# OPPOMKLab/u-LLaVA

Hardware: AMD Instinct MI355X
Metric: images/sec/GPU (ViT-L-336 + LLaMA-7B + SAM RES forward) at 1/2/4/8 MI355X (higher is better)
Workload: dtype bf16; 1 GPU; C4: ViT-L/14-336 + LLaMA-7B instruct forward, 336x336 image + 64-token prompt (S=643), batch 32/GPU; per_gpu_batch=32, global_batch=32, seq_len=643, image=336, parallelism=dp1, weights=random-init N(0,0.02), ViT-L/14 + LLaMA-7B (V=32011) shapes

## Files before the change

### u-llava_amd/csrc/gemm.hip

```cpp
#include "ull_common.h"
#include <stdlib.h>
#include <type_traits>

namespace {

constexpr int BM = 128, BN = 128, BK = 64;
constexpr int TILE_BYTES = BM * BK * 2;
constexpr int BUF_BYTES = 2 * TILE_BYTES;
constexpr int GEMM_LDS = 2 * BUF_BYTES;
constexpr int GROUP_M = 8;

constexpr int EPI_BIAS = 1, EPI_ACT_SHIFT = 1, EPI_ACT_MASK = 3 << 1;
constexpr int EPI_RESID = 8, EPI_SWIGLU = 16, EPI_OUT_F32 = 32;
constexpr int EPI_W_TILED = 64, EPI_X_TILED = 128;
constexpr int EPI_BIAS_ROUNDED = 256;
constexpr int ULL_W4_FORCE_STAGED = 512;

struct GemmArgs {
    const elem_t* X; const elem_t* W; void* C;
    const elem_t* bias; const elem_t* R;
    long ldx, ldw, ldc, ldr;
    int M, N, K, flags;
    int nbm, nbn;
    int t_full, sk;
// ... 733 lines not shown
    __builtin_amdgcn_s_barrier();
    staged_epilogue<SWIGLU, 4>(p, acc, smem + wave * (64 * 144), lane, m0 + wm * 64, n0 + wn * 64);
}
#endif


struct PatchArgs {
    const elem_t* img; const elem_t* zeros; const elem_t* img_end;
    int C, H, W, ps, gw, gh;
    int nseg;
    int xcd_raster;
};

template <int DUMMY>
__global__ __launch_bounds__(256, 2) void patchify_gemm_kernel(GemmArgs p, PatchArgs q) {
    extern __shared__ __attribute__((aligned(16))) char smem[];
    const int tid = threadIdx.x;
    const int lane = tid & 63;
    const int wave = __builtin_amdgcn_readfirstlane(tid >> 6);
    const int wn = wave & 1, wm = wave >> 1;
    const int nwg = p.nbm * p.nbn;
    int bid = blockIdx.x;
    {
        const int qq = nwg >> 3, r = nwg & 7, xcd = bid & 7, k = bid >> 3;
        bid = (xcd < r ? xcd * (qq + 1) : r * (qq + 1) + (xcd - r) * qq) + k;
    }
    const int per_group = GROUP_M * p.nbn;
    const int gid = bid / per_group;
    const int first_m = gid * GROUP_M;
    const int gsz = min(p.nbm - first_m, GROUP_M);
    const int bm = first_m + (bid % per_group) % gsz;
    const int bn = (bid % per_group) / gsz;
    const int m0 = bm * BM, n0 = bn * BN;

    const int srow = lane >> 3;
    const int schunk = (lane & 7) ^ srow;
    const int seg = schunk >> 1, half = schunk & 1;
    const elem_t* xbase[4];
    const elem_t* wsrc[4];
#pragma unroll
    for (int i = 0; i < 4; ++i) {
        const int r = (wave * 4 + i) * 8 + srow;
        const int m = min(m0 + r, p.M - 1);
        const int px = m % q.gw, py = (m / q.gw) % q.gh, b = m / (q.gw * q.gh);
        xbase[i] = q.img + (((long)b * q.C * q.H + (long)py * q.ps) * q.W + px * q.ps) + half * 8;
        wsrc[i] = p.W + (long)min(n0 + r, p.N - 1) * p.ldw + schunk * 8;
    }
    const int stage_off = wave * 4 * 8 * (BK * 2);
    const uint32_t lds_base = __builtin_amdgcn_readfirstlane((uint32_t)(uintptr_t)(__attribute__((address_space(3))) char*)smem);
    auto stage = [&](int buf, int kt) {
        const uint32_t bx = lds_base + buf * BUF_BYTES + stage_off;
        const uint32_t bw = bx + TILE_BYTES;
        const int idx = kt * 4 + seg;
        const int c = idx / q.ps, ky = idx - c * q.ps;
        const long xoff = ((long)c * q.H + ky) * q.W;
        const bool real = idx < q.nseg;
        const long ko = (long)kt * BK;
#pragma unroll
        for (int i = 0; i < 4; ++i) {
            const elem_t* sp = real ? xbase[i] + xoff : q.zeros;
            if (real && sp + 8 > q.img_end) {
                const uint32_t* s32 = (const uint32_t*)sp;
                const uint4 v = make_uint4(s32[0], s32[1], s32[2], 0u);
                *(uint4*)(smem + buf * BUF_BYTES + stage_off + i * 1024 + lane * 16) = v;
                asm volatile("s_waitcnt lgkmcnt(0)" ::: "memory");
            } else {
                glds16(sp, bx + i * 1024);
            }
            glds16(wsrc[i] + ko, bw + i * 1024);
        }
    };

    const int frow = lane & 15, fgrp = lane >> 4;
    int swz[2];
    swz[0] = ((0 + fgrp) ^ (lane & 7)) << 4;
    swz[1] = ((4 + fgrp) ^ (lane & 7)) << 4;
    const int xrow_off = (wm * 64 + frow) * (BK * 2);
    const int wrow_off = TILE_BYTES + (wn * 64 + frow) * (BK * 2);

    f32x4_t acc[4][4];
#pragma unroll
    for (int i = 0; i < 4; ++i)
#pragma unroll
        for (int j = 0; j < 4; ++j) acc[i][j] = f32x4_t{0.f, 0.f, 0.f, 0.f};

    const int nk = p.K / BK;
    stage(0, 0);
    for (int kt = 0; kt < nk; ++kt) {
        const int cur = kt & 1;
        asm volatile("s_waitcnt vmcnt(0)" ::: "memory");
        __builtin_amdgcn_s_barrier();
        if (kt + 1 < nk) stage(cur ^ 1, kt + 1);
        const char* base = smem + cur * BUF_BYTES;
#pragma unroll
        for (int kk = 0; kk < 2; ++kk) {
            uint4 wf[4], xf[4];
#pragma unroll
            for (int i = 0; i < 4; ++i) wf[i] = *(const uint4*)(base + wrow_off + i * 16 * (BK * 2) + swz[kk]);
#pragma unroll
            for (int j = 0; j < 4; ++j) xf[j] = *(const uint4*)(base + xrow_off + j * 16 * (BK * 2) + swz[kk]);
#pragma unroll
            for (int i = 0; i < 4; ++i)
#pragma unroll
                for (int j = 0; j < 4; ++j) acc[i][j] = mfma16(wf[i], xf[j], acc[i][j]);
        }
    }
    __builtin_amdgcn_s_barrier();
    staged_epilogue<false, 4>(p, acc, smem + wave * (64 * 144), lane, m0 + wm * 64, n0 + wn * 64);
}

#define ULL_STAMP(slot) ((void)0)

namespace big {

constexpr int BM = 256, BN = 256, BK = 64;
constexpr int OP_BYTES = BM * BK * 2;
constexpr int SLOT_BYTES = 2 * OP_BYTES;
constexpr int LDS_BYTES = 8 * 128 * (64 * 2 + 16);
constexpr int LDS_BYTES_W4 = LDS_BYTES + 16 * 1024;

struct Frags { uint4 w[4]; uint4 x[8]; };

template <bool SWIGLU, bool ROPE = false>
__global__ __launch_bounds__(512) void gemm256_kernel(GemmArgs p) {
    extern __shared__ __attribute__((aligned(16))) char smem[];
    const int tid = threadIdx.x, lane = tid & 63;
    const int wave = __builtin_amdgcn_readfirstlane(tid >> 6);
    const int wn = wave & 3, wm = wave >> 2;
    int bid = blockIdx.x;
    int slice = 0;
    const bool split = bid >= p.t_full;
    if (!split) {
        const int nwg = p.t_full;
        const int q = nwg >> 3, r = nwg & 7, xcd = bid & 7, k = bid >> 3;
        bid = (xcd < r ? xcd * (q + 1) : r * (q + 1) + (xcd - r) * q) + k;
    } else {
        const int r = bid - p.t_full;
        bid = p.t_full + r / p.sk;
        slice = r % p.sk;
    }
    const int per_group = p.group_m * p.nbn;
    const int gid = bid / per_group;
    const int first_m = gid * p.group_m;
    const int gsz = min(p.nbm - first_m, p.group_m);
    const int bm = first_m + (bid % per_group) % gsz;
    const int bn = (bid % per_group) / gsz;
    const int m0 = bm * BM, n0 = bn * BN;
    const int nk_total = p.K / BK;
    const bool w_tiled = p.flags & EPI_W_TILED, x_tiled = p.flags & EPI_X_TILED;

    const int srow = lane >> 3;
    const int schunk = (lane & 7) ^ srow;
    const elem_t* xsrc[4];
    const elem_t* wsrc[4];
#pragma unroll
    for (int i = 0; i < 4; ++i) {
        const int r = (wave * 4 + i) * 8 + srow;
        xsrc[i] = x_tiled ? p.X + (((long)bm * nk_total) * BM + r) * BK + schunk * 8
                          : p.X + (long)min(m0 + r, p.M - 1) * p.ldx + schunk * 8;
        wsrc[i] = w_tiled ? p.W + (((long)bn * nk_total) * BN + r) * BK + schunk * 8
                          : p.W + (long)min(n0 + r, p.N - 1) * p.ldw + schunk * 8;
    }
    const long xstep = x_tiled ? BM * BK : BK, wstep = w_tiled ? BN * BK : BK;
    const uint32_t lds_base = __builtin_amdgcn_readfirstlane((uint32_t)(uintptr_t)(__attribute__((address_space(3))) char*)smem);
    const uint32_t piece_off = wave * 4 * 1024;
    auto stage = [&](int kt) {
        const uint32_t bx = lds_base + (kt & 1) * SLOT_BYTES + piece_off;
        const long kox = (long)kt * xstep, kow = (long)kt * wstep;
#pragma unroll
        for (int i = 0; i < 4; ++i) {
            glds16(xsrc[i] + kox, bx + i * 1024);
            glds16(wsrc[i] + kow, bx + OP_BYTES + i * 1024);
        }
    };

    const int fr = lane & 15, fg = lane >> 4;
    int swz[2];
    swz[0] = ((0 + fg) ^ (lane & 7)) << 4;
    swz[1] = ((4 + fg) ^ (lane & 7)) << 4;
    const int xoff = (wm * 128 + fr) * (BK * 2);
    const int woff = OP_BYTES + (wn * 64 + fr) * (BK * 2);
    auto read_frags = [&](int kt, int kk, Frags& f) {
        const char* base = smem + (kt & 1) * SLOT_BYTES + swz[kk];
#pragma unroll
        for (int i = 0; i < 4; ++i) f.w[i] = *(const uint4*)(base + woff + i * 16 * (BK * 2));
#pragma unroll
        for (int j = 0; j < 8; ++j) f.x[j] = *(const uint4*)(base + xoff + j * 16 * (BK * 2));
    };

    f32x4_t acc[4][8];
#pragma unroll
    for (int i = 0; i < 4; ++i)
#pragma unroll
        for (int j = 0; j < 8; ++j) acc[i][j] = f32x4_t{0.f, 0.f, 0.f, 0.f};
    int nk = p.K / BK;
    if (split) {
        const int kt0 = (int)((long)nk * slice / p.sk), kt1 = (int)((long)nk * (slice + 1) / p.sk);
#pragma unroll
        for (int i = 0; i < 4; ++i) { xsrc[i] += (long)kt0 * xstep; wsrc[i] += (long)kt0 * wstep; }
        nk = kt1 - kt0;
    }
constexpr int ULL_W8_BAR_A = 14;
constexpr int ULL_W8_DMA_STRIDE = 6;
constexpr int ULL_W8_BAR_B = 40;
constexpr int ULL_W8_FA_STRIDE = 2;
    constexpr int W8_BAR_A = ULL_W8_BAR_A, W8_DMA_STRIDE = ULL_W8_DMA_STRIDE, W8_BAR_B = ULL_W8_BAR_B, W8_FA_STRIDE = ULL_W8_FA_STRIDE;
    constexpr int W8_ISSUED = (W8_BAR_B - W8_BAR_A + W8_DMA_STRIDE - 1) / W8_DMA_STRIDE;
    constexpr int W8_INFLIGHT = W8_ISSUED > 8 ? 8 : W8_ISSUED;
    static_assert(W8_BAR_A >= 12 && W8_BAR_B >= W8_BAR_A && W8_BAR_A + 7 * W8_DMA_STRIDE < 64 && W8_BAR_B + 11 * W8_FA_STRIDE < 64, "schedule");
    constexpr int USE_ORDER[12] = {0, 4, 1, 2, 3, 5, 6, 7, 8, 9, 10, 11};
    auto read1 = [&](int kt, int kk, Frags& f, int r) {
        const char* base = smem + (kt & 1) * SLOT_BYTES + swz[kk];
        if (r < 4) f.w[r] = *(const uint4*)(base + woff + r * 16 * (BK * 2));
        else f.x[r - 4] = *(const uint4*)(base + xoff + (r - 4) * 16 * (BK * 2));
    };
    auto mma1 = [&](const Frags& f, int s) {
        const int j = s >> 2, i = s & 3;
        acc[i][j] = mfma16(f.w[i], f.x[j], acc[i][j]);
    };
    stage(0);
    stage(1);
    asm volatile("s_waitcnt vmcnt(8)" ::: "memory");
    __builtin_amdgcn_s_barrier();
    Frags fa, fb;
    read_frags(0, 0, fa);
    const uint32_t dump = lds_base + LDS_BYTES;
#pragma clang loop unroll(disable)
    for (int kt = 0; kt < nk; ++kt) {
        const bool with_dma = kt + 2 < nk;
        const int ktd = with_dma ? kt + 2 : nk - 1;
        const long kox = (long)ktd * xstep, kow = (long)ktd * wstep;
        const uint32_t bx = with_dma ? lds_base + (kt & 1) * SLOT_BYTES + piece_off : dump;
        const uint32_t bw = with_dma ? bx + OP_BYTES : dump + 4096;
#pragma clang loop unroll(full)
        for (int s = 0; s < 64; ++s) {
            if (s == W8_BAR_A) {
                asm volatile("s_waitcnt lgkmcnt(0)" ::: "memory");
                __builtin_amdgcn_s_barrier();
            }
            if (s == W8_BAR_B) {
                asm volatile("s_waitcnt vmcnt(%0)" :: "n"(W8_INFLIGHT) : "memory");
                __builtin_amdgcn_s_barrier();
            }
            if (s < 12) read1(kt, 1, fb, s);
            if (s >= W8_BAR_B && (s - W8_BAR_B) % W8_FA_STRIDE == 0 && (s - W8_BAR_B) / W8_FA_STRIDE < 12)
                read1(kt + 1, 0, fa, USE_ORDER[(s - W8_BAR_B) / W8_FA_STRIDE]);
            if (s >= W8_BAR_A && (s - W8_BAR_A) % W8_DMA_STRIDE == 0 && (s - W8_BAR_A) / W8_DMA_STRIDE < 8) {
                const int pc = (s - W8_BAR_A) / W8_DMA_STRIDE;
                if (pc < 4) glds16(xsrc[pc] + kox, bx + pc * 1024);
                else glds16(wsrc[pc - 4] + kow, bw + (pc - 4) * 1024);
            }
            mma1(s < 32 ? fa : fb, s & 31);
            __builtin_amdgcn_sched_barrier(0);
        }
    }

    if (split) {
        float* slab = p.ws + ((long)(bid - p.t_full) * p.sk + slice) * (BM * BN);
#pragma clang loop unroll(full)
        for (int j = 0; j < 8; ++j)
#pragma clang loop unroll(full)
            for (int i = 0; i < 4; ++i)
                *(f32x4_t*)(slab + (wm * 128 + j * 16 + fr) * BN + wn * 64 + i * 16 + fg * 4) = acc[i][j];
        return;
    }
    __builtin_amdgcn_s_barrier();
    staged_epilogue<SWIGLU, 8, ROPE>(p, acc, smem + wave * (128 * 144), lane, m0 + wm * 128, n0 + wn * 64, smem + (wave ^ 1) * (128 * 144));
}


struct Frags4 { uint4 w[8]; uint4 x[8]; };

#ifdef ULL_ELEM_F16
#define ULL_MFMA16_ASM "v_mfma_f32_16x16x32_f16"
#else
#define ULL_MFMA16_ASM "v_mfma_f32_16x16x32_bf16"
#endif
typedef uint32_t u32x4_t __attribute__((ext_vector_type(4)));
ULL_DEV void mfma16_inplace(f32x4_t& c, const uint4& a, const uint4& b) {
    const u32x4_t av = {a.x, a.y, a.z, a.w}, bv = {b.x, b.y, b.z, b.w};
    asm volatile(ULL_MFMA16_ASM " %0, %1, %2, %0" : "+a"(c) : "v"(av), "v"(bv));
}


template <bool SWIGLU> ULL_DEV int w4_row_swizzle(int row) {
    return SWIGLU ? (((row >> 1) & 1) | (((row >> 3) & 1) << 1) | (((row >> 5) & 1) << 2)) : (((row >> 1) & 1) | (((row >> 3) & 3) << 1));
}
template <bool SWIGLU> ULL_DEV constexpr int w4_frag_row(int c) {
    return SWIGLU ? 64 * (c >> 2) + 16 * (c & 1) + 4 * ((c >> 1) & 1) : 32 * (c >> 1) + 4 * (c & 1);
}
template <bool SWIGLU> ULL_DEV int w4_lane_row(int fr) {
    return SWIGLU ? 32 * (fr >> 3) + 8 * ((fr >> 2) & 1) + (fr & 3) : 8 * (fr >> 2) + (fr & 3);
}
template <bool SWIGLU> ULL_DEV int w4_acc_row(int h, int i, int fg) {
    return SWIGLU ? h * 64 + 32 * (fg >> 1) + 16 * (i & 1) + 8 * (fg & 1) + 4 * (i >> 1) : h * 64 + 32 * (i >> 1) + 8 * fg + 4 * (i & 1);
}

ULL_DEV f32x4_t w4_acc_to_vgpr(const f32x4_t& a) {
    f32x4_t t = a;
    asm volatile("" : "+v"(t));
    return t;
}

template <bool SWIGLU, bool ROPE, int NH = 2, int RPF = 8>
ULL_DEV void w4_direct_epilogue(const GemmArgs& p, f32x4_t (&acc)[NH][4][8], int lane, int mrow0, int nw0) {
    static_assert(NH == 2 || (!SWIGLU && !ROPE), "SwiGLU and RoPE pair columns across the two halves");
    const int fr = lane & 15, fg = lane >> 4;
    if constexpr (SWIGLU) {
        const int n_out = p.N / 2, nb = nw0 / 2 + 8 * fg;
        elem_t* cb = (elem_t*)p.C + nb;
#pragma clang loop unroll(full)
        for (int j = 0; j < 8; ++j) {
            const int m = mrow0 + j * 16 + fr;
#pragma clang loop unroll(full)
            for (int h = 0; h < 2; ++h) {
                float v[8];
#pragma clang loop unroll(full)
                for (int pp = 0; pp < 2; ++pp) {
                    const f32x4_t ag = w4_acc_to_vgpr(acc[h][2 * pp][j]), au = w4_acc_to_vgpr(acc[h][2 * pp + 1][j]);
#pragma unroll
                    for (int r = 0; r < 4; ++r) {
                        const float g = rnd(ag[r]);
                        const float u = rnd(au[r]);
                        v[4 * pp + r] = rnd(act_silu(g)) * u;
                    }
                }
                if (m < p.M && nb + h * 32 + 8 <= n_out) *(uint4*)(cb + (long)m * p.ldc + h * 32) = pack8(v);
            }
            __builtin_amdgcn_sched_barrier(0);
        }
    } else {
        const int flags = p.flags;
        const bool has_bias = flags & EPI_BIAS, has_res = flags & EPI_RESID;
        const bool rope_on = ROPE && nw0 < p.rope_cols;
        const int nb = nw0 + 8 * fg;
        uint4 bvp[NH][2];
#pragma unroll
        for (int h = 0; h < NH; ++h)
#pragma unroll
            for (int pp = 0; pp < 2; ++pp) {
                const int n = nb + h * 64 + pp * 32;
                bvp[h][pp] = (has_bias && n + 8 <= p.N) ? *(const uint4*)(p.bias + n) : uint4{0, 0, 0, 0};
            }
        elem_t* cb = (elem_t*)p.C + nb;
        const elem_t* rb = p.R + nb;
        auto body = [&](auto with_bias, auto with_res, auto act_kind) {
            constexpr bool WB = decltype(with_bias)::value, WR = decltype(with_res)::value;
            constexpr int ACT = decltype(act_kind)::value;
            constexpr int NB_ = ROPE ? 2 : RPF;
            uint4 rv[NB_][NH][2], tc[NB_][2], ts[NB_][2];
            auto fetch = [&](int j, int buf) {
                const long mc = min(mrow0 + j * 16 + fr, p.M - 1);
                if constexpr (WR) {
#pragma unroll
                    for (int h = 0; h < NH; ++h)
#pragma unroll
                        for (int pp = 0; pp < 2; ++pp) rv[buf][h][pp] = *(const uint4*)(rb + mc * p.ldr + h * 64 + pp * 32);
                }
                if constexpr (ROPE) {
                    if (rope_on) {
#pragma unroll
                        for (int pp = 0; pp < 2; ++pp) {
                            tc[buf][pp] = *(const uint4*)(p.rope_cos + mc * 64 + pp * 32 + 8 * fg);
                            ts[buf][pp] = *(const uint4*)(p.rope_sin + mc * 64 + pp * 32 + 8 * fg);
                        }
                    }
                }
            };
            if constexpr (ROPE || NB_ < 8) fetch(0, 0);
            else if constexpr (WR) {
#pragma clang loop unroll(full)
                for (int j = 0; j < 8; ++j) fetch(j, j);
                __builtin_amdgcn_sched_barrier(0);
            }
#pragma clang loop unroll(full)
            for (int j = 0; j < 8; ++j) {
                const int m = mrow0 + j * 16 + fr;
                if constexpr (ROPE || NB_ < 8) { if (j + 1 < 8) fetch(j + 1, (j + 1) % NB_); }
                uint4 o[NH][2];
#pragma unroll
                for (int h = 0; h < NH; ++h)
#pragma unroll
                    for (int pp = 0; pp < 2; ++pp) {
                        float v[8], bv[8];
                        if constexpr (WB) unpack8(bvp[h][pp], bv);
                        const f32x4_t a0 = w4_acc_to_vgpr(acc[h][2 * pp][j]), a1 = w4_acc_to_vgpr(acc[h][2 * pp + 1][j]);
#pragma unroll
                        for (int e = 0; e < 8; ++e) {
                            const float a = e < 4 ? a0[e & 3] : a1[e & 3];
                            v[e] = WB ? a + bv[e] : a;
                        }
                        o[h][pp] = pack8(v);
                        if constexpr (ACT != 0) {
                            float a[8];
                            unpack8(o[h][pp], a);
                            if constexpr (ACT == 2) {
#pragma unroll
                                for (int e = 0; e < 8; e += 2) {
                                    const f32x2_t r = act_gelu_erf2(f32x2_t{a[e], a[e + 1]});
                                    a[e] = r.x; a[e + 1] = r.y;
                                }
                            } else {
#pragma unroll
                                for (int e = 0; e < 8; ++e) a[e] = ACT == 1 ? act_quick_gelu_e(a[e]) : fmaxf(a[e], 0.f);
                            }
                            o[h][pp] = pack8(a);
                        }
                    }
                if constexpr (ROPE) {
                    if (rope_on) {
#pragma unroll
                        for (int pp = 0; pp < 2; ++pp) {
                            float x0[8], x1[8], cs[8], sn[8];
                            unpack8(o[0][pp], x0); unpack8(o[1][pp], x1);
                            unpack8(tc[j % NB_][pp], cs); unpack8(ts[j % NB_][pp], sn);
                            float y0[8], y1[8];
#pragma unroll
                            for (int e = 0; e < 8; ++e) {
                                y0[e] = rnd(x0[e] * cs[e]) + rnd(-x1[e] * sn[e]);
                                y1[e] = rnd(x1[e] * cs[e]) + rnd(x0[e] * sn[e]);
                            }
                            o[0][pp] = pack8(y0); o[1][pp] = pack8(y1);
                        }
                    }
                }
#pragma unroll
                for (int h = 0; h < NH; ++h)
#pragma unroll
                    for (int pp = 0; pp < 2; ++pp) {
                        if constexpr (WR) {
                            float a[8], b[8];
                            unpack8(o[h][pp], a); unpack8(rv[j % NB_][h][pp], b);
#pragma unroll
                            for (int e = 0; e < 8; ++e) a[e] = rnd(b[e] + a[e]);
                            o[h][pp] = pack8(a);
                        }
                        if (m < p.M && nb + h * 64 + pp * 32 + 8 <= p.N) *(uint4*)(cb + (long)m * p.ldc + h * 64 + pp * 32) = o[h][pp];
                    }
                __builtin_amdgcn_sched_barrier(0);
            }
        };
        using I0 = std::integral_constant<int, 0>;
        const int act = (flags & EPI_ACT_MASK) >> EPI_ACT_SHIFT;
        if constexpr (!ROPE) {
            if (act) {
                if (act == 1) { if (has_bias) body(std::true_type{}, std::false_type{}, std::integral_constant<int, 1>{}); else body(std::false_type{}, std::false_type{}, std::integral_constant<int, 1>{}); }
                else if (act == 2) { if (has_bias) body(std::true_type{}, std::false_type{}, std::integral_constant<int, 2>{}); else body(std::false_type{}, std::false_type{}, std::integral_constant<int, 2>{}); }
                else { if (has_bias) body(std::true_type{}, std::false_type{}, std::integral_constant<int, 3>{}); else body(std::false_type{}, std::false_type{}, std::integral_constant<int, 3>{}); }
                return;
            }
        }
        if (has_bias) { if (has_res) body(std::true_type{}, std::true_type{}, I0{}); else body(std::true_type{}, std::false_type{}, I0{}); }
        else { if (has_res) body(std::false_type{}, std::true_type{}, I0{}); else body(std::false_type{}, std::false_type{}, I0{}); }
    }
}

template <bool SWIGLU, bool ROPE = false>
__global__ __launch_bounds__(256) void gemm256w4_kernel(GemmArgs p) {
    extern __shared__ __attribute__((aligned(16))) char smem[];
    ULL_STAMP(0); ULL_STAMP(7);
    const int tid = threadIdx.x, lane = tid & 63;
    const int wave = __builtin_amdgcn_readfirstlane(tid >> 6);
    const int wn = wave & 1, wm = wave >> 1;
    int bid = blockIdx.x;
    int slice = 0;
    const bool split = bid >= p.t_full;
    if (!split) {
        const int nwg = p.t_full;
        const int q = nwg >> 3, r = nwg & 7, xcd = bid & 7, k = bid >> 3;
        bid = (xcd < r ? xcd * (q + 1) : r * (q + 1) + (xcd - r) * q) + k;
    } else {
        const int r = bid - p.t_full;
        bid = p.t_full + r / p.sk;
        slice = r % p.sk;
    }
    const int per_group = p.group_m * p.nbn;
    const int gid = bid / per_group;
    const int first_m = gid * p.group_m;
    const int gsz = min(p.nbm - first_m, p.group_m);
    const int bm = first_m + (bid % per_group) % gsz;
    const int bn = (bid % per_group) / gsz;
    const int m0 = bm * BM, n0 = bn * BN;
    const int nk_total = p.K / BK;
    const bool w_tiled = p.flags & EPI_W_TILED, x_tiled = p.flags & EPI_X_TILED;

    const int srow = lane >> 3;
    const int schunk = (lane & 7) ^ srow;
    uint32_t xo[8], wo[8];
#pragma unroll
    for (int i = 0; i < 8; ++i) {
        const int r = (wave * 8 + i) * 8 + srow;
        const int wchunk = (lane & 7) ^ w4_row_swizzle<SWIGLU>(r);
        xo[i] = x_tiled ? (uint32_t)(r * BK + schunk * 8) * 2 : (uint32_t)(((long)(min(m0 + r, p.M - 1) - m0) * p.ldx + schunk * 8) * 2);
        wo[i] = w_tiled ? (uint32_t)(r * BK + wchunk * 8) * 2 : (uint32_t)(((long)(min(n0 + r, p.N - 1) - n0) * p.ldw + wchunk * 8) * 2);
    }
    const elem_t* xbase = x_tiled ? p.X + ((long)bm * nk_total) * BM * BK : p.X + (long)m0 * p.ldx;
    const elem_t* wbase = w_tiled ? p.W + ((long)bn * nk_total) * BN * BK : p.W + (long)n0 * p.ldw;
    const long xstep = x_tiled ? BM * BK : BK, wstep = w_tiled ? BN * BK : BK;
    const uint32_t lds_base = __builtin_amdgcn_readfirstlane((uint32_t)(uintptr_t)(__attribute__((address_space(3))) char*)smem);
    const uint32_t piece_off = wave * 8 * 1024;
    auto dma_piece = [&](const elem_t* xk, const elem_t* wk, uint32_t slot_addr, int c) {
        if (c < 8) glds16s(xk, xo[c], slot_addr + c * 1024);
        else glds16s(wk, wo[c - 8], slot_addr + OP_BYTES + (c - 8) * 1024);
    };
    auto stage_all = [&](int kt) {
        const elem_t* xk = xbase + (long)kt * xstep;
        const elem_t* wk = wbase + (long)kt * wstep;
        const uint32_t sa = lds_base + (kt & 1) * SLOT_BYTES + piece_off;
#pragma unroll
        for (int c = 0; c < 16; ++c) dma_piece(xk, wk, sa, c);
    };

    const int fr = lane & 15, fg = lane >> 4;
    int swz[2];
    swz[0] = ((0 + fg) ^ (lane & 7)) << 4;
    swz[1] = ((4 + fg) ^ (lane & 7)) << 4;
    int wswz[2];
    wswz[0] = ((0 + fg) ^ (fr >> 1)) << 4;
    wswz[1] = ((4 + fg) ^ (fr >> 1)) << 4;
    const int xoff = (wm * 128 + fr) * (BK * 2);
    const int woff = OP_BYTES + (wn * 128 + w4_lane_row<SWIGLU>(fr)) * (BK * 2);
    auto read_one = [&](int kt, int kk, Frags4& f, int c) {
        const char* base = smem + (kt & 1) * SLOT_BYTES;
        if (c < 8) f.w[c] = *(const uint4*)(base + wswz[kk] + woff + w4_frag_row<SWIGLU>(c) * (BK * 2));
        else f.x[c - 8] = *(const uint4*)(base + swz[kk] + xoff + (c - 8) * 16 * (BK * 2));
    };

    f32x4_t acc[2][4][8];
#pragma unroll
    for (int h = 0; h < 2; ++h)
#pragma unroll
        for (int i = 0; i < 4; ++i)
#pragma unroll
            for (int j = 0; j < 8; ++j) acc[h][i][j] = f32x4_t{0.f, 0.f, 0.f, 0.f};
    auto chunk_mma = [&](const Frags4& f, int c) {
        const int j = c >> 1, h = c & 1;
#pragma unroll
        for (int i = 0; i < 4; ++i) mfma16_inplace(acc[h][i][j], f.w[h * 4 + i], f.x[j]);
    };

    int nk = p.K / BK;
    if (split) {
        const int kt0 = (int)((long)nk * slice / p.sk), kt1 = (int)((long)nk * (slice + 1) / p.sk);
        xbase += (long)kt0 * xstep; wbase += (long)kt0 * wstep;
        nk = kt1 - kt0;
    }
    ULL_STAMP(1);
    stage_all(0);
    stage_all(1);
    asm volatile("s_waitcnt vmcnt(16)" ::: "memory");
    __builtin_amdgcn_s_barrier();
    ULL_STAMP(2);
    Frags4 fa, fb;
#pragma unroll
    for (int c = 0; c < 16; ++c) read_one(0, 0, fa, c);
constexpr int ULL_W4_BAR_A = 20;
constexpr int ULL_W4_BAR_B = 96;
constexpr int ULL_W4_FB_STRIDE = 1;
constexpr int ULL_W4_FA_FIRST = 96;
constexpr int ULL_W4_FA_STRIDE = 2;
constexpr int ULL_W4_DMA_FIRST = 20;
constexpr int ULL_W4_DMA_STRIDE = 7;
    constexpr int W4_BAR_A = ULL_W4_BAR_A, W4_BAR_B = ULL_W4_BAR_B, W4_FB_STRIDE = ULL_W4_FB_STRIDE, W4_FA_FIRST = ULL_W4_FA_FIRST,
                  W4_FA_STRIDE = ULL_W4_FA_STRIDE, W4_DMA_FIRST = ULL_W4_DMA_FIRST, W4_DMA_STRIDE = ULL_W4_DMA_STRIDE;
    constexpr int W4_ISSUED = (W4_BAR_B - W4_DMA_FIRST + W4_DMA_STRIDE - 1) / W4_DMA_STRIDE;
    constexpr int W4_INFLIGHT = W4_ISSUED < 0 ? 0 : W4_ISSUED > 16 ? 16 : W4_ISSUED;
    static_assert(W4_BAR_A >= 15 * W4_FB_STRIDE + 1 && W4_DMA_FIRST >= W4_BAR_A && W4_FA_FIRST >= W4_BAR_B, "schedule order");
    static_assert(W4_DMA_FIRST + 15 * W4_DMA_STRIDE < 128 && W4_FA_FIRST + 15 * W4_FA_STRIDE < 128, "schedule fits the step");
    constexpr int USE_ORDER[16] = {0, 8, 1, 2, 3, 4, 5, 6, 7, 9, 10, 11, 12, 13, 14, 15};
    auto slot_mma = [&](const Frags4& f, int s) {
        const int j = s >> 3, h = (s >> 2) & 1, i = s & 3;
        mfma16_inplace(acc[h][i][j], f.w[h * 4 + i], f.x[j]);
    };
    auto slot_mma_dma = [&](const Frags4& f, int s, const void* sbase, uint32_t voff, uint32_t lds_addr) {
        const int j = s >> 3, h = (s >> 2) & 1, i = s & 3;
        const uint4 &a = f.w[h * 4 + i], &b = f.x[j];
        const u32x4_t av = {a.x, a.y, a.z, a.w}, bv = {b.x, b.y, b.z, b.w};
        asm volatile("s_mov_b32 m0, %5\n\t" ULL_MFMA16_ASM " %0, %1, %2, %0\n\tglobal_load_lds_dwordx4 %3, %4"
                     : "+a"(acc[h][i][j]) : "v"(av), "v"(bv), "v"(voff), "s"(sbase), "s"(lds_addr) : "memory");
    };
    uint32_t m0_keep;
    asm volatile("s_mov_b32 %0, m0" : "=s"(m0_keep));
    const uint32_t dump = lds_base + LDS_BYTES;
#pragma clang loop unroll(disable)
    for (int kt = 0; kt < nk; ++kt) {
        const bool with_dma = kt + 2 < nk;
        const int ktd = with_dma ? kt + 2 : nk - 1;
        const elem_t* xk = xbase + (long)ktd * xstep;
        const elem_t* wk = wbase + (long)ktd * wstep;
        const uint32_t sa = with_dma ? lds_base + (kt & 1) * SLOT_BYTES + piece_off : dump;
        const uint32_t sw = with_dma ? sa + OP_BYTES : dump;
#pragma clang loop unroll(full)
        for (int s = 0; s < 128; ++s) {
            if (s == W4_BAR_A) {
                asm volatile("s_waitcnt lgkmcnt(0)" ::: "memory");
                __builtin_amdgcn_s_barrier();
            }
            if (s == W4_BAR_B) {
                asm volatile("s_waitcnt vmcnt(%0)" :: "n"(W4_INFLIGHT) : "memory");
                __builtin_amdgcn_s_barrier();
            }
            if (s < 16 * W4_FB_STRIDE && s % W4_FB_STRIDE == 0) read_one(kt, 1, fb, s / W4_FB_STRIDE);
            if (s >= W4_FA_FIRST && (s - W4_FA_FIRST) % W4_FA_STRIDE == 0 && (s - W4_FA_FIRST) / W4_FA_STRIDE < 16)
                read_one(kt + 1, 0, fa, USE_ORDER[(s - W4_FA_FIRST) / W4_FA_STRIDE]);
            const Frags4& f = s < 64 ? fa : fb;
            const int pc = (s - W4_DMA_FIRST) / W4_DMA_STRIDE;
            if (s >= W4_DMA_FIRST && (s - W4_DMA_FIRST) % W4_DMA_STRIDE == 0 && pc < 16) {
                if (pc < 8) slot_mma_dma(f, s & 63, xk, xo[pc], sa + pc * 1024);
                else slot_mma_dma(f, s & 63, wk, wo[pc - 8], sw + (pc - 8) * 1024);
            } else slot_mma(f, s & 63);
            __builtin_amdgcn_sched_barrier(0);
        }
        if (kt == nk - 1) asm volatile("s_nop 15\n\ts_nop 7" ::: "memory");
    }
    ULL_STAMP(3);
    asm volatile("s_mov_b32 m0, %0" :: "s"(m0_keep) : "memory");

    if (split) {
        float* slab = p.ws + ((long)(bid - p.t_full) * p.sk + slice) * (BM * BN);
#pragma clang loop unroll(full)
        for (int j = 0; j < 8; ++j)
#pragma clang loop unroll(full)
            for (int h = 0; h < 2; ++h)
#pragma clang loop unroll(full)
                for (int i = 0; i < 4; ++i)
                    *(f32x4_t*)(slab + (wm * 128 + j * 16 + fr) * BN + wn * 128 + w4_acc_row<SWIGLU>(h, i, fg)) = acc[h][i][j];
        return;
    }
    const int mrow0 = m0 + wm * 128, nw0 = n0 + wn * 128;
    {
        const int fl = p.flags;
        const bool direct = ROPE || (!(fl & (EPI_OUT_F32 | EPI_BIAS_ROUNDED)) && (!(fl & EPI_ACT_MASK) || !(fl & EPI_RESID)) && (p.ldc & 7) == 0 &&
                                     ((SWIGLU ? p.N / 2 : p.N) & 7) == 0 && (!(fl & EPI_RESID) || (p.ldr & 7) == 0) && !(fl & ULL_W4_FORCE_STAGED));
        if (direct) {
            w4_direct_epilogue<SWIGLU, ROPE>(p, acc, lane, mrow0, nw0);
            ULL_STAMP(4);
            asm volatile("s_waitcnt vmcnt(0)" ::: "memory");
            ULL_STAMP(5);
            return;
        }
    }
    __builtin_amdgcn_s_barrier();
    char* reg0 = smem + wave * (2 * 128 * 144);
    if constexpr (ROPE) {
        return;
    } else if constexpr (SWIGLU) {
        staged_epilogue<true, 8, false, 1, true, 4, true, 1>(p, acc[0], reg0, lane, mrow0, nw0, nullptr, 0);
        staged_epilogue<true, 8, false, 1, true, 4, true, 1>(p, acc[1], reg0, lane, mrow0, nw0, nullptr, 1);
        staged_epilogue<true, 8, false, 2, true, 4, true, 1>(p, acc[0], reg0, lane, mrow0, nw0);
    } else {
#pragma clang loop unroll(disable)
        for (int h = 0; h < 2; ++h) {
            if (h == 0) staged_epilogue<false, 8, false, 1, true, 4, false, 1>(p, acc[0], reg0, lane, mrow0, nw0);
            else staged_epilogue<false, 8, false, 1, true, 4, false, 1>(p, acc[1], reg0, lane, mrow0, nw0 + 64);
            staged_epilogue<false, 8, false, 2, true, 4, false, 1>(p, acc[0], reg0, lane, mrow0, nw0 + 64 * h);
        }
    }
}


template <int WMB>
__global__ __launch_bounds__(512) void patchify_strip_kernel(GemmArgs p, PatchArgs q) {
    extern __shared__ __attribute__((aligned(16))) char smem[];
    constexpr int TM = 32 * WMB, TN = 256;
    constexpr int A_BYTES = TM * 128, W_BYTES = TN * 128, STAGE = A_BYTES + W_BYTES;
    constexpr int NPIECE = (TM + TN) / 8;
    const int tid = threadIdx.x, lane = tid & 63;
    const int wave = __builtin_amdgcn_readfirstlane(tid >> 6);
    const int wn = wave & 3, wm = wave >> 2;
    const int fr = lane & 15, fg = lane >> 4;
    int bn = blockIdx.x % p.nbn, bm = blockIdx.x / p.nbn;
    if (q.xcd_raster) {
        const int xcd = blockIdx.x & 7, slot = blockIdx.x >> 3;
        bm = xcd * (p.nbm >> 3) + slot / p.nbn;
        bn = slot % p.nbn;
    }
    const int m0 = bm * TM, n0 = bn * TN;
    const int srow = lane >> 3;
    const uint32_t lds_base = __builtin_amdgcn_readfirstlane((uint32_t)(uintptr_t)(__attribute__((address_space(3))) char*)smem);
    constexpr int PPW = (NPIECE + 7) / 8;
    int* segtab = (int*)(smem + 2 * STAGE);
    if (tid < 64) {
        const int c = tid / q.ps, ky = tid - c * q.ps;
        segtab[tid] = tid < q.nseg ? (c * q.H + ky) * q.W : -1;
    }
    const elem_t* src[PPW];
    const int schunk = (lane & 7) ^ srow;
    const int aseg = schunk >> 1;
#pragma unroll
    for (int i = 0; i < PPW; ++i) {
        const int pc = wave + 8 * i;
        src[i] = nullptr;
        if (pc < TM / 8) {
            const int r = pc * 8 + srow;
            const int m = min(m0 + r, p.M - 1);
            const int px = m % q.gw, py = (m / q.gw) % q.gh, b = m / (q.gw * q.gh);
            src[i] = q.img + (((long)b * q.C * q.H + (long)py * q.ps) * q.W + px * q.ps) + (schunk & 1) * 8;
        } else if (pc < NPIECE) {
            const int r = (pc - TM / 8) * 8 + srow;
            const int wchunk = (lane & 7) ^ w4_row_swizzle<false>(r);
            src[i] = p.W + (long)min(n0 + r, p.N - 1) * p.ldw + wchunk * 8;
        }
    }
    const bool tail_strip = __builtin_amdgcn_readfirstlane(m0 + TM >= p.M ? 1 : 0) != 0;
    __syncthreads();
    auto stage_t = [&](int buf, int kt, auto guarded) {
        const uint32_t sb = lds_base + buf * STAGE;
        const int off = segtab[kt * 4 + aseg];
#pragma unroll
        for (int i = 0; i < PPW; ++i) {
            const int pc = wave + 8 * i;
            if (pc >= NPIECE) continue;
            if (pc < TM / 8) {
                const elem_t* sp = off >= 0 ? src[i] + off : q.zeros;
                if (decltype(guarded)::value && off >= 0 && sp + 8 > q.img_end) {
                    const uint32_t* s32 = (const uint32_t*)sp;
                    *(uint4*)(smem + buf * STAGE + pc * 1024 + lane * 16) = make_uint4(s32[0], s32[1], s32[2], 0u);
                    asm volatile("s_waitcnt lgkmcnt(0)" ::: "memory");
                } else {
                    glds16(sp, sb + pc * 1024);
                }
            } else {
                glds16(src[i] + (long)kt * BK, sb + A_BYTES + (pc - TM / 8) * 1024);
            }
        }
    };
    auto stage = [&](int buf, int kt) {
        if (tail_strip) stage_t(buf, kt, std::true_type{});
        else stage_t(buf, kt, std::false_type{});
    };
    int swz[2], wswz[2];
    swz[0] = ((0 + fg) ^ (lane & 7)) << 4;
    swz[1] = ((4 + fg) ^ (lane & 7)) << 4;
    wswz[0] = ((0 + fg) ^ (fr >> 1)) << 4;
    wswz[1] = ((4 + fg) ^ (fr >> 1)) << 4;
    const int xoff = (wm * 16 * WMB + fr) * 128;
    const int woff = A_BYTES + (wn * 64 + w4_lane_row<false>(fr)) * 128;

    f32x4_t acc[4][WMB];
#pragma unroll
    for (int i = 0; i < 4; ++i)
#pragma unroll
        for (int j = 0; j < WMB; ++j) acc[i][j] = f32x4_t{0.f, 0.f, 0.f, 0.f};
    const int nk = p.K / BK;
    stage(0, 0);
    for (int kt = 0; kt < nk; ++kt) {
        const int cur = kt & 1;
        asm volatile("s_waitcnt vmcnt(0)" ::: "memory");
        __builtin_amdgcn_s_barrier();
        if (kt + 1 < nk) stage(cur ^ 1, kt + 1);
        const char* base = smem + cur * STAGE;
#pragma unroll
        for (int kk = 0; kk < 2; ++kk) {
            uint4 wf[4], xf[WMB];
#pragma unroll
            for (int i = 0; i < 4; ++i) wf[i] = *(const uint4*)(base + wswz[kk] + woff + w4_frag_row<false>(i) * 128);
#pragma unroll
            for (int j = 0; j < WMB; ++j) xf[j] = *(const uint4*)(base + swz[kk] + xoff + j * 16 * 128);
#pragma unroll
            for (int j = 0; j < WMB; ++j)
#pragma unroll
                for (int i = 0; i < 4; ++i) acc[i][j] = mfma16(wf[i], xf[j], acc[i][j]);
        }
    }
    const int nb = n0 + wn * 64 + 8 * fg;
    float bv[2][8];
#pragma unroll
    for (int pp = 0; pp < 2; ++pp) {
        if ((p.flags & EPI_BIAS) && nb + pp * 32 + 8 <= p.N) unpack8(*(const uint4*)(p.bias + nb + pp * 32), bv[pp]);
        else {
#pragma unroll
            for (int e = 0; e < 8; ++e) bv[pp][e] = -0.0f;
        }
    }
    elem_t* cb = (elem_t*)p.C + nb;
#pragma unroll
    for (int j = 0; j < WMB; ++j) {
        const int m = m0 + wm * 16 * WMB + j * 16 + fr;
#pragma unroll
        for (int pp = 0; pp < 2; ++pp) {
            float v[8];
#pragma unroll
            for (int e = 0; e < 8; ++e) v[e] = acc[2 * pp + (e >> 2)][j][e & 3] + bv[pp][e];
            if (m < p.M && nb + pp * 32 + 8 <= p.N) *(uint4*)(cb + (long)m * p.ldc + pp * 32) = pack8(v);
        }
    }
}

__global__ __launch_bounds__(512) void gemm256d_kernel(GemmArgs p) {
    constexpr bool SWIGLU = false, ROPE = false;
    extern __shared__ __attribute__((aligned(16))) char smem[];
    const int tid = threadIdx.x, lane = tid & 63;
    const int wave = __builtin_amdgcn_readfirstlane(tid >> 6);
    const int wn = wave & 3, wm = wave >> 2;
    int bid = blockIdx.x;
    int slice = 0;
    const bool split = bid >= p.t_full;
    if (!split) {
        const int nwg = p.t_full;
        const int q = nwg >> 3, r = nwg & 7, xcd = bid & 7, k = bid >> 3;
        bid = (xcd < r ? xcd * (q + 1) : r * (q + 1) + (xcd - r) * q) + k;
    } else {
        const int r = bid - p.t_full;
        bid = p.t_full + r / p.sk;
        slice = r % p.sk;
    }
    const int per_group = p.group_m * p.nbn;
    const int gid = bid / per_group;
    const int first_m = gid * p.group_m;
    const int gsz = min(p.nbm - first_m, p.group_m);
    const int bm = first_m + (bid % per_group) % gsz;
    const int bn = (bid % per_group) / gsz;
    const int m0 = bm * BM, n0 = bn * BN;
    const int nk_total = p.K / BK;
    const bool w_tiled = p.flags & EPI_W_TILED, x_tiled = p.flags & EPI_X_TILED;

    const int srow = lane >> 3;
    const int schunk = (lane & 7) ^ srow;
    const elem_t* xsrc[4];
    const elem_t* wsrc[4];
#pragma unroll
    for (int i = 0; i < 4; ++i) {
        const int r = (wave * 4 + i) * 8 + srow;
        xsrc[i] = x_tiled ? p.X + (((long)bm * nk_total) * BM + r) * BK + schunk * 8
                          : p.X + (long)min(m0 + r, p.M - 1) * p.ldx + schunk * 8;
        const int wchunk = (lane & 7) ^ w4_row_swizzle<false>(r);
        wsrc[i] = w_tiled ? p.W + (((long)bn * nk_total) * BN + r) * BK + wchunk * 8
                          : p.W + (long)min(n0 + r, p.N - 1) * p.ldw + wchunk * 8;
    }
    const long xstep = x_tiled ? BM * BK : BK, wstep = w_tiled ? BN * BK : BK;
    const uint32_t lds_base = __builtin_amdgcn_readfirstlane((uint32_t)(uintptr_t)(__attribute__((address_space(3))) char*)smem);
    const uint32_t piece_off = wave * 4 * 1024;
    auto stage = [&](int kt) {
        const uint32_t bx = lds_base + (kt & 1) * SLOT_BYTES + piece_off;
        const long kox = (long)kt * xstep, kow = (long)kt * wstep;
#pragma unroll
        for (int i = 0; i < 4; ++i) {
            glds16(xsrc[i] + kox, bx + i * 1024);
            glds16(wsrc[i] + kow, bx + OP_BYTES + i * 1024);
        }
    };

    const int fr = lane & 15, fg = lane >> 4;
    int swz[2];
    swz[0] = ((0 + fg) ^ (lane & 7)) << 4;
    swz[1] = ((4 + fg) ^ (lane & 7)) << 4;
    int wswz[2];
    wswz[0] = ((0 + fg) ^ (fr >> 1)) << 4;
    wswz[1] = ((4 + fg) ^ (fr >> 1)) << 4;
    const int xoff = (wm * 128 + fr) * (BK * 2);
    const int woff = OP_BYTES + (wn * 64 + w4_lane_row<false>(fr)) * (BK * 2);
    auto read_frags = [&](int kt, int kk, Frags& f) {
        const char* base = smem + (kt & 1) * SLOT_BYTES;
#pragma unroll
        for (int i = 0; i < 4; ++i) f.w[i] = *(const uint4*)(base + wswz[kk] + woff + w4_frag_row<false>(i) * (BK * 2));
#pragma unroll
        for (int j = 0; j < 8; ++j) f.x[j] = *(const uint4*)(base + swz[kk] + xoff + j * 16 * (BK * 2));
    };

    f32x4_t acc[1][4][8];
#pragma unroll
    for (int i = 0; i < 4; ++i)
#pragma unroll
        for (int j = 0; j < 8; ++j) acc[0][i][j] = f32x4_t{0.f, 0.f, 0.f, 0.f};
    int nk = p.K / BK;
    if (split) {
        const int kt0 = (int)((long)nk * slice / p.sk), kt1 = (int)((long)nk * (slice + 1) / p.sk);
#pragma unroll
        for (int i = 0; i < 4; ++i) { xsrc[i] += (long)kt0 * xstep; wsrc[i] += (long)kt0 * wstep; }
        nk = kt1 - kt0;
    }
constexpr int ULL_W8_BAR_A = 14;
constexpr int ULL_W8_DMA_STRIDE = 6;
constexpr int ULL_W8_BAR_B = 40;
constexpr int ULL_W8_FA_STRIDE = 2;
    constexpr int W8_BAR_A = ULL_W8_BAR_A, W8_DMA_STRIDE = ULL_W8_DMA_STRIDE, W8_BAR_B = ULL_W8_BAR_B, W8_FA_STRIDE = ULL_W8_FA_STRIDE;
    constexpr int W8_ISSUED = (W8_BAR_B - W8_BAR_A + W8_DMA_STRIDE - 1) / W8_DMA_STRIDE;
    constexpr int W8_INFLIGHT = W8_ISSUED > 8 ? 8 : W8_ISSUED;
    static_assert(W8_BAR_A >= 12 && W8_BAR_B >= W8_BAR_A && W8_BAR_A + 7 * W8_DMA_STRIDE < 64 && W8_BAR_B + 11 * W8_FA_STRIDE < 64, "schedule");
    constexpr int USE_ORDER[12] = {0, 4, 1, 2, 3, 5, 6, 7, 8, 9, 10, 11};
    auto read1 = [&](int kt, int kk, Frags& f, int r) {
        const char* base = smem + (kt & 1) * SLOT_BYTES;
        if (r < 4) f.w[r] = *(const uint4*)(base + wswz[kk] + woff + w4_frag_row<false>(r) * (BK * 2));
        else f.x[r - 4] = *(const uint4*)(base + swz[kk] + xoff + (r - 4) * 16 * (BK * 2));
    };
    auto mma1 = [&](const Frags& f, int s) {
        const int j = s >> 2, i = s & 3;
        acc[0][i][j] = mfma16(f.w[i], f.x[j], acc[0][i][j]);
    };
    stage(0);
    stage(1);
    asm volatile("s_waitcnt vmcnt(8)" ::: "memory");
    __builtin_amdgcn_s_barrier();
    Frags fa, fb;
    read_frags(0, 0, fa);
    const uint32_t dump = lds_base + LDS_BYTES;
#pragma clang loop unroll(disable)
    for (int kt = 0; kt < nk; ++kt) {
        const bool with_dma = kt + 2 < nk;
        const int ktd = with_dma ? kt + 2 : nk - 1;
        const long kox = (long)ktd * xstep, kow = (long)ktd * wstep;
        const uint32_t bx = with_dma ? lds_base + (kt & 1) * SLOT_BYTES + piece_off : dump;
        const uint32_t bw = with_dma ? bx + OP_BYTES : dump + 4096;
#pragma clang loop unroll(full)
        for (int s = 0; s < 64; ++s) {
            if (s == W8_BAR_A) {
                asm volatile("s_waitcnt lgkmcnt(0)" ::: "memory");
                __builtin_amdgcn_s_barrier();
            }
            if (s == W8_BAR_B) {
                asm volatile("s_waitcnt vmcnt(%0)" :: "n"(W8_INFLIGHT) : "memory");
                __builtin_amdgcn_s_barrier();
            }
            if (s < 12) read1(kt, 1, fb, s);
            if (s >= W8_BAR_B && (s - W8_BAR_B) % W8_FA_STRIDE == 0 && (s - W8_BAR_B) / W8_FA_STRIDE < 12)
                read1(kt + 1, 0, fa, USE_ORDER[(s - W8_BAR_B) / W8_FA_STRIDE]);
            if (s >= W8_BAR_A && (s - W8_BAR_A) % W8_DMA_STRIDE == 0 && (s - W8_BAR_A) / W8_DMA_STRIDE < 8) {
                const int pc = (s - W8_BAR_A) / W8_DMA_STRIDE;
                if (pc < 4) glds16(xsrc[pc] + kox, bx + pc * 1024);
                else glds16(wsrc[pc - 4] + kow, bw + (pc - 4) * 1024);
            }
            mma1(s < 32 ? fa : fb, s & 31);
            __builtin_amdgcn_sched_barrier(0);
        }
    }

    if (split) {
        float* slab = p.ws + ((long)(bid - p.t_full) * p.sk + slice) * (BM * BN);
#pragma clang loop unroll(full)
        for (int j = 0; j < 8; ++j)
#pragma clang loop unroll(full)
            for (int i = 0; i < 4; ++i)
                *(f32x4_t*)(slab + (wm * 128 + j * 16 + fr) * BN + wn * 64 + w4_acc_row<false>(0, i, fg)) = acc[0][i][j];
        return;
    }
    {
        const int fl = p.flags;
        const bool direct = !(fl & (EPI_OUT_F32 | EPI_BIAS_ROUNDED)) && (!(fl & EPI_ACT_MASK) || !(fl & EPI_RESID)) && (p.ldc & 7) == 0 && (p.N & 7) == 0 &&
// ... 368 lines not shown
```

Before: 145.4 images/sec (whole job, all GPUs).

## Prefetch RoPE cos/sin tables into LDS during last GEMM k-steps; reorder prologue DMA

In the RoPE variant of the W4 GEMM kernel, the final two k-iterations' dummy DMA slots now asynchronously load the rope cos/sin rows into the free LDS slot, so the epilogue reads them from LDS instead of global memory. The prologue is also restructured so the first X-tile DMA is issued before the W offsets are computed, which hides address arithmetic behind the load. This removes global-memory latency from the fused QKV+RoPE epilogue at the cost of a more intricate two-phase k-loop with pointer-arithmetic slot selection.

```diff
diff --git a/u-llava_amd/csrc/gemm.hip b/u-llava_amd/csrc/gemm.hip
--- a/u-llava_amd/csrc/gemm.hip
+++ b/u-llava_amd/csrc/gemm.hip
@@ -1059,8 +1059,10 @@
     return t;
 }
 
+typedef const __attribute__((address_space(3))) char* lds_cptr_t;
+constexpr int W4_ROPE_SIN_OFF = 128 * 128;
 template <bool SWIGLU, bool ROPE, int NH = 2, int RPF = 8>
-ULL_DEV void w4_direct_epilogue(const GemmArgs& p, f32x4_t (&acc)[NH][4][8], int lane, int mrow0, int nw0) {
+ULL_DEV void w4_direct_epilogue(const GemmArgs& p, f32x4_t (&acc)[NH][4][8], int lane, int mrow0, int nw0, lds_cptr_t rope_lds = nullptr) {
     static_assert(NH == 2 || (!SWIGLU && !ROPE), "SwiGLU and RoPE pair columns across the two halves");
     const int fr = lane & 15, fg = lane >> 4;
     if constexpr (SWIGLU) {
@@ -1118,8 +1120,11 @@
                     if (rope_on) {
 #pragma unroll
                         for (int pp = 0; pp < 2; ++pp) {
-                            tc[buf][pp] = *(const uint4*)(p.rope_cos + mc * 64 + pp * 32 + 8 * fg);
-                            ts[buf][pp] = *(const uint4*)(p.rope_sin + mc * 64 + pp * 32 + 8 * fg);
+                            const int off = (j * 16 + fr) * 128 + (((4 * pp + fg) ^ (fr >> 1)) << 4);
+                            const u32x4_t c = *(const __attribute__((address_space(3))) u32x4_t*)(rope_lds + off);
+                            const u32x4_t sv = *(const __attribute__((address_space(3))) u32x4_t*)(rope_lds + W4_ROPE_SIN_OFF + off);
+                            tc[buf][pp] = uint4{c.x, c.y, c.z, c.w};
+                            ts[buf][pp] = uint4{sv.x, sv.y, sv.z, sv.w};
                         }
                     }
                 }
@@ -1243,30 +1248,57 @@
 
     const int srow = lane >> 3;
     const int schunk = (lane & 7) ^ srow;
-    uint32_t xo[8], wo[8];
-#pragma unroll
-    for (int i = 0; i < 8; ++i) {
-        const int r = (wave * 8 + i) * 8 + srow;
-        const int wchunk = (lane & 7) ^ w4_row_swizzle<SWIGLU>(r);
-        xo[i] = x_tiled ? (uint32_t)(r * BK + schunk * 8) * 2 : (uint32_t)(((long)(min(m0 + r, p.M - 1) - m0) * p.ldx + schunk * 8) * 2);
-        wo[i] = w_tiled ? (uint32_t)(r * BK + wchunk * 8) * 2 : (uint32_t)(((long)(min(n0 + r, p.N - 1) - n0) * p.ldw + wchunk * 8) * 2);
-    }
     const elem_t* xbase = x_tiled ? p.X + ((long)bm * nk_total) * BM * BK : p.X + (long)m0 * p.ldx;
     const elem_t* wbase = w_tiled ? p.W + ((long)bn * nk_total) * BN * BK : p.W + (long)n0 * p.ldw;
     const long xstep = x_tiled ? BM * BK : BK, wstep = w_tiled ? BN * BK : BK;
     const uint32_t lds_base = __builtin_amdgcn_readfirstlane((uint32_t)(uintptr_t)(__attribute__((address_space(3))) char*)smem);
     const uint32_t piece_off = wave * 8 * 1024;
+    int nk = nk_total;
+    if (split) {
+        const int kt0 = (int)((long)nk * slice / p.sk), kt1 = (int)((long)nk * (slice + 1) / p.sk);
+        xbase += (long)kt0 * xstep; wbase += (long)kt0 * wstep;
+        nk = kt1 - kt0;
+    }
+    uint32_t xo[8], wo[8];
+    if (x_tiled) {
+#pragma unroll
+        for (int i = 0; i < 8; ++i) xo[i] = (uint32_t)(((wave * 8 + i) * 8 + srow) * BK + schunk * 8) * 2;
+    } else {
+#pragma unroll
+        for (int i = 0; i < 8; ++i) xo[i] = (uint32_t)(((long)(min(m0 + (wave * 8 + i) * 8 + srow, p.M - 1) - m0) * p.ldx + schunk * 8) * 2);
+    }
     auto dma_piece = [&](const elem_t* xk, const elem_t* wk, uint32_t slot_addr, int c) {
         if (c < 8) glds16s(xk, xo[c], slot_addr + c * 1024);
         else glds16s(wk, wo[c - 8], slot_addr + OP_BYTES + (c - 8) * 1024);
     };
-    auto stage_all = [&](int kt) {
+    auto stage_range = [&](int kt, int c0, int c1) {
         const elem_t* xk = xbase + (long)kt * xstep;
         const elem_t* wk = wbase + (long)kt * wstep;
         const uint32_t sa = lds_base + (kt & 1) * SLOT_BYTES + piece_off;
 #pragma unroll
-        for (int c = 0; c < 16; ++c) dma_piece(xk, wk, sa, c);
-    };
+        for (int c = c0; c < c1; ++c) dma_piece(xk, wk, sa, c);
+    };
+    ULL_STAMP(1);
+    __builtin_amdgcn_sched_barrier(0);
+    stage_range(0, 0, 8);
+    __builtin_amdgcn_sched_barrier(0);
+    if (w_tiled) {
+#pragma unroll
+        for (int i = 0; i < 8; ++i) {
+            const int r = (wave * 8 + i) * 8 + srow;
+            wo[i] = (uint32_t)(r * BK + ((lane & 7) ^ w4_row_swizzle<SWIGLU>(r)) * 8) * 2;
+        }
+    } else {
+#pragma unroll
+        for (int i = 0; i < 8; ++i) {
+            const int r = (wave * 8 + i) * 8 + srow;
+            wo[i] = (uint32_t)(((long)(min(n0 + r, p.N - 1) - n0) * p.ldw + ((lane & 7) ^ w4_row_swizzle<SWIGLU>(r)) * 8) * 2);
+        }
+    }
+    __builtin_amdgcn_sched_barrier(0);
+    stage_range(0, 8, 16);
+    stage_range(1, 0, 16);
+    __builtin_amdgcn_sched_barrier(0);
 
     const int fr = lane & 15, fg = lane >> 4;
     int swz[2];
@@ -1296,15 +1328,6 @@
         for (int i = 0; i < 4; ++i) mfma16_inplace(acc[h][i][j], f.w[h * 4 + i], f.x[j]);
     };
 
-    int nk = p.K / BK;
-    if (split) {
-        const int kt0 = (int)((long)nk * slice / p.sk), kt1 = (int)((long)nk * (slice + 1) / p.sk);
-        xbase += (long)kt0 * xstep; wbase += (long)kt0 * wstep;
-        nk = kt1 - kt0;
-    }
-    ULL_STAMP(1);
-    stage_all(0);
-    stage_all(1);
     asm volatile("s_waitcnt vmcnt(16)" ::: "memory");
     __builtin_amdgcn_s_barrier();
     ULL_STAMP(2);
@@ -1339,14 +1362,7 @@
     uint32_t m0_keep;
     asm volatile("s_mov_b32 %0, m0" : "=s"(m0_keep));
     const uint32_t dump = lds_base + LDS_BYTES;
-#pragma clang loop unroll(disable)
-    for (int kt = 0; kt < nk; ++kt) {
-        const bool with_dma = kt + 2 < nk;
-        const int ktd = with_dma ? kt + 2 : nk - 1;
-        const elem_t* xk = xbase + (long)ktd * xstep;
-        const elem_t* wk = wbase + (long)ktd * wstep;
-        const uint32_t sa = with_dma ? lds_base + (kt & 1) * SLOT_BYTES + piece_off : dump;
-        const uint32_t sw = with_dma ? sa + OP_BYTES : dump;
+    auto step = [&](int kt, const elem_t* xk, const elem_t* wk, uint32_t sa, uint32_t sw) {
 #pragma clang loop unroll(full)
         for (int s = 0; s < 128; ++s) {
             if (s == W4_BAR_A) {
@@ -1369,6 +1385,54 @@
             __builtin_amdgcn_sched_barrier(0);
         }
         if (kt == nk - 1) asm volatile("s_nop 15\n\ts_nop 7" ::: "memory");
+    };
+    if constexpr (!ROPE) {
+#pragma clang loop unroll(disable)
+        for (int kt = 0; kt < nk; ++kt) {
+            const bool with_dma = kt + 2 < nk;
+            const int ktd = with_dma ? kt + 2 : nk - 1;
+            const elem_t* xk = xbase + (long)ktd * xstep;
+            const elem_t* wk = wbase + (long)ktd * wstep;
+            const uint32_t sa = with_dma ? lds_base + (kt & 1) * SLOT_BYTES + piece_off : dump;
+            const uint32_t sw = with_dma ? sa + OP_BYTES : dump;
+            step(kt, xk, wk, sa, sw);
+        }
+    } else {
+        const bool rope_stage = !split && n0 < p.rope_cols;
+#pragma clang loop unroll(disable)
+        for (int ph = 0; ph < 2; ++ph) {
+            int kt = 0, hi = nk - 2;
+            const elem_t* xk = xbase + 2 * xstep;
+            const elem_t* wk = wbase + 2 * wstep;
+            long xs = xstep, ws = wstep;
+            uint32_t sa0 = lds_base + piece_off, sw0 = sa0 + OP_BYTES, sad = SLOT_BYTES, swd = SLOT_BYTES;
+            if (ph) {
+                kt = nk - 2; hi = nk;
+                xs = ws = 0;
+                sa0 = sw0 = dump; sad = swd = 0;
+                xk = xbase + (long)(nk - 1) * xstep;
+                wk = wbase + (long)(nk - 1) * wstep;
+                if (rope_stage) {
+                    const int mrow0_s = m0 + wm * 128, rb = min(mrow0_s, p.M - 1);
+                    xk = wk = (wn ? p.rope_sin : p.rope_cos) + (long)rb * 64;
+#pragma unroll
+                    for (int i = 0; i < 16; ++i) {
+                        const uint32_t o = (uint32_t)(min(mrow0_s + 8 * i + srow, p.M - 1) - rb) * 128 +
+                                           (uint32_t)(((lane & 7) ^ ((4 * i + (lane >> 4)) & 7)) << 4);
+                        if (i < 8) xo[i] = o; else wo[i - 8] = o;
+                    }
+                    const uint32_t ra = lds_base + (nk & 1) * SLOT_BYTES + wave * (16 * 1024);
+                    if (nk & 1) { sad = ra - dump; swd = sad + 8 * 1024; }
+                    else { sa0 = ra; sw0 = ra + 8 * 1024; sad = dump - sa0; swd = dump - sw0; }
+                }
+            }
+#pragma clang loop unroll(disable)
+            for (; kt < hi; ++kt) {
+                const uint32_t odd = (uint32_t)-(kt & 1);
+                step(kt, xk, wk, sa0 + (sad & odd), sw0 + (swd & odd));
+                xk += xs; wk += ws;
+            }
+        }
     }
     ULL_STAMP(3);
     asm volatile("s_mov_b32 m0, %0" :: "s"(m0_keep) : "memory");
@@ -1390,7 +1454,8 @@
         const bool direct = ROPE || (!(fl & (EPI_OUT_F32 | EPI_BIAS_ROUNDED)) && (!(fl & EPI_ACT_MASK) || !(fl & EPI_RESID)) && (p.ldc & 7) == 0 &&
                                      ((SWIGLU ? p.N / 2 : p.N) & 7) == 0 && (!(fl & EPI_RESID) || (p.ldr & 7) == 0) && !(fl & ULL_W4_FORCE_STAGED));
         if (direct) {
-            w4_direct_epilogue<SWIGLU, ROPE>(p, acc, lane, mrow0, nw0);
+            w4_direct_epilogue<SWIGLU, ROPE>(p, acc, lane, mrow0, nw0,
+                                             (lds_cptr_t)(__attribute__((address_space(3))) char*)smem + (nk & 1) * SLOT_BYTES + wm * (32 * 1024));
             ULL_STAMP(4);
             asm volatile("s_waitcnt vmcnt(0)" ::: "memory");
             ULL_STAMP(5);
```

Measured after the change: 146.4 images/sec (whole job, all GPUs), median of 6. About the same (+0.7%).
